# Chrixtar/latentsplat

Hardware: AMD Instinct MI355X
Metric: rendered target views/sec at 256x256, ~300k Gaussians (forward); fwd+bwd ms/view in `fwdbwd` (higher is better)
Workload: dtype f32; 1 GPU; BASELINE configs[1]: 300000 latent Gaussians (4-ch features + opacity), 256x256, forward render; 16 views of one scene per step per GPU; gaussians=300000, parallelism=replicas x1 (one scene per rank, no data-path collective)

## Files before the change

### latentsplat_amd/csrc/binning.hip

```cpp
#include "lsr_blend.h"
#include "lsr_tile_scan.h"
#include <algorithm>
#include <mutex>
#ifdef LSR_ENABLE_TRACE
#include <cstdio>
#include <cstdlib>
#include <vector>
#endif

namespace lsr {

constexpr int kScanThreads = 1024;

constexpr int kScanRegs = 8;

__global__ void __launch_bounds__(kScanThreads)
k_tile_scan(const uint32_t *__restrict__ count, uint32_t *__restrict__ start, uint32_t *header,
            uint32_t *host_words, uint32_t host_seq, uint32_t *__restrict__ order, int N, uint32_t capacity) {
    __shared__ TileScanShared<kScanThreads> s_scan;
    tile_scan_block<kScanThreads, kScanRegs, false>(count, start, header, HostMirror{host_words, host_seq}, order, N, capacity, s_scan);
}

hipError_t launch_tile_scan(const lsr_dims &d, char *geom, uint32_t *host_words, uint32_t host_seq, uint32_t pair_capacity, hipStream_t s) {
    const GeomLayout L = geom_layout(d);
// ... 107 lines not shown
    if (trace && threadIdx.x == 0) {
        unsigned hwid, xcc;
        asm volatile("s_getreg_b32 %0, hwreg(HW_REG_HW_ID)" : "=s"(hwid));
        asm volatile("s_getreg_b32 %0, hwreg(HW_REG_XCC_ID)" : "=s"(xcc));
        trace[8 * (size_t)blockIdx.x + 7] = ((unsigned long long)(xcc & 0xff) << 32) | hwid;
    }
#endif
#undef LSR_STAMP
}

constexpr int kSortThreads = 512;

struct HalfOut {
    uint32_t *half_list, *half_count;
    uint32_t *header;
    uint32_t capacity;
    uint32_t *long_list;
    uint32_t long_cap;
    uint32_t *long_count[2];
    IndexPacking ip;
    uint32_t seg_cap;
    const uint64_t *seg_keys;
    uint32_t n_limit;
};
constexpr int kSortTier2 = 8192;
__device__ __forceinline__ uint32_t long_tile(const HalfOut &ho, int cls, uint32_t i) {
    return ho.long_list[cls ? ho.long_cap - 1u - i : i];
}
__device__ __forceinline__ uint32_t key_index(const HalfOut &ho, uint32_t low_word) { return low_word >> ho.ip.key_shift; }
__device__ __forceinline__ uint32_t key_mask(const HalfOut &ho, uint32_t low_word) { return ho.ip.key_shift ? code_mask(low_word & 0xFFu) : 0xFFFFu; }
__device__ __forceinline__ uint32_t list_entry(const HalfOut &ho, uint32_t idx, uint32_t bits) { return idx | ((bits << kListBitsShift) & ~ho.ip.index_mask); }
constexpr int kEmitTab = 130;

template <int THREADS, class LowWord>
__device__ __forceinline__ void emit_half_lists(const HalfOut &ho, uint32_t n, uint32_t *hdst, uint32_t *hcnt, uint64_t *s_tab, LowWord low_word) {
    const int tid = threadIdx.x, lane = tid & (LSR_WAVE - 1), wid = tid / LSR_WAVE;
    constexpr int kWaves = THREADS / LSR_WAVE;
    uint32_t run0 = 0u, run1 = 0u;
    for (uint32_t base = 0; base < n; base += LSR_WAVE * LSR_WAVE) {
        for (int c = wid; c < LSR_WAVE; c += kWaves) {
            const uint32_t p = base + (uint32_t)(c * LSR_WAVE + lane);
            uint64_t packed = 0;
            if (p - lane < n) {
                const uint32_t w = low_word(min(p, n - 1));
                const uint32_t m16 = p < n ? key_mask(ho, w) : 0u;
                packed = (uint64_t)__builtin_popcountll(__ballot((m16 & 0x00FFu) != 0u)) |
                         ((uint64_t)__builtin_popcountll(__ballot((m16 & 0xFF00u) != 0u)) << 32);
            }
            if (lane == 0) s_tab[c] = packed;
        }
        __syncthreads();
        if (wid == 0) {
            const uint64_t v = s_tab[lane];
            uint64_t incl = v;
#pragma unroll
            for (int off = 1; off < LSR_WAVE; off <<= 1) { const uint64_t t = __shfl_up(incl, off); if (lane >= off) incl += t; }
            s_tab[LSR_WAVE + lane] = incl - v;
            if (lane == LSR_WAVE - 1) s_tab[2 * LSR_WAVE] = incl;
        }
        __syncthreads();
        const uint64_t tot = s_tab[2 * LSR_WAVE];
        for (int c = wid; c < LSR_WAVE; c += kWaves) {
            const uint32_t p = base + (uint32_t)(c * LSR_WAVE + lane);
            if (p - lane >= n) break;
            const uint32_t w = low_word(min(p, n - 1));
            const uint32_t idx = key_index(ho, w), m16 = p < n ? key_mask(ho, w) : 0u;
            const uint64_t off = s_tab[LSR_WAVE + c];
#pragma unroll
            for (int h = 0; h < 2; ++h) {
                const uint32_t bits = half_bits(m16, h);
                const uint64_t bal = __ballot(bits != 0u);
                if (bits) {
                    const uint32_t below = __builtin_amdgcn_mbcnt_hi((uint32_t)(bal >> 32), __builtin_amdgcn_mbcnt_lo((uint32_t)bal, 0u));
                    hdst[(size_t)h * n + (h ? run1 : run0) + (uint32_t)(off >> (32 * h)) + below] = list_entry(ho, idx, bits);
                }
            }
        }
        run0 += (uint32_t)tot; run1 += (uint32_t)(tot >> 32);
        __syncthreads();
    }
    if (tid < 2) hcnt[tid] = tid == 0 ? run0 : run1;
}

constexpr uint32_t kBucketOverflow = 48;

template <int CAP, int THREADS>
__device__ __forceinline__ void sort_tile(uint64_t *s_keys, size_t vt, int tier, const uint32_t *__restrict__ tile_start,
                                          const uint64_t *__restrict__ keys, uint32_t *__restrict__ point_list,
                                          const HalfOut &ho, unsigned long long *trace) {
#ifdef LSR_ENABLE_TRACE
#define LSR_STAMP(k) do { if (trace && threadIdx.x == 0) trace[8 * (size_t)blockIdx.x + (k)] = wall_clock64(); } while (0)
#else
#define LSR_STAMP(k) do { } while (0)
#endif
    LSR_STAMP(0);
    static_assert(CAP % THREADS == 0, "whole keys per thread");
    constexpr int NB = CAP < 2048 ? CAP : 2048;
    constexpr int kWaves = THREADS / LSR_WAVE;
    uint32_t *s_cnt = (uint32_t *)(s_keys + CAP);
    uint64_t *s_red = s_keys;
    uint32_t *s_wsum = (uint32_t *)(s_keys + 2 * kWaves);
    uint32_t *s_flag = s_wsum + kWaves;
    const int tid = threadIdx.x, lane = tid & (LSR_WAVE - 1), wid = tid / LSR_WAVE;
    const uint32_t start = tile_start[vt], n = tile_start[vt + 1] - start;
    uint32_t *hcnt = ho.half_count + 2 * vt, *hdst = ho.half_list + 2 * (size_t)start;
    if (n == 0) { if (tid < 2) hcnt[tid] = 0; return; }
    if ((uint64_t)start + n > ho.capacity) {
        if (tid < 2) hcnt[tid] = 0;
        if (tid == 0) ho.header[kHdrOverflow] = 1u;
        return;
    }
    if (n > ho.n_limit) {
        if (tid < 2) hcnt[tid] = 0;
        return;
    }
    if (n > (uint32_t)CAP) {
        if (tid == 0 && tier == 0) {
            const int cls = n > (uint32_t)kSortTier2 ? 1 : 0;
            const uint32_t i = atomicAdd(ho.long_count[cls], 1u);
            ho.long_list[cls ? ho.long_cap - 1u - i : i] = (uint32_t)vt;
        }
        return;
    }
    const uint64_t *src = (ho.seg_cap && n <= ho.seg_cap) ? ho.seg_keys + vt * (size_t)ho.seg_cap : keys + start;
    if (n == 1) {
        if (tid == 0) {
            const uint32_t w = (uint32_t)src[0], idx = key_index(ho, w);
            point_list[start] = idx;
            const uint32_t m = key_mask(ho, w);
            for (int h = 0; h < 2; ++h) {
                const uint32_t bits = half_bits(m, h);
                if (bits) hdst[h] = list_entry(ho, idx, bits);
                hcnt[h] = bits ? 1u : 0u;
            }
        }
        return;
    }

    constexpr int PERK = CAP / THREADS;
    uint64_t kreg[PERK];
#pragma unroll
    for (int q = 0; q < PERK; ++q) {
        const uint32_t i = tid + q * THREADS;
        const uint64_t k = src[min(i, n - 1)];
        kreg[q] = i < n ? k : ~0ull;
    }
    uint64_t kmin = ~0ull, kmax = 0ull;
#pragma unroll
    for (int q = 0; q < PERK; ++q) {
        const uint64_t k = kreg[q];
        kmin = k < kmin ? k : kmin;
        if (tid + q * THREADS < n) kmax = k > kmax ? k : kmax;
    }
#pragma unroll
    for (int off = 32; off > 0; off >>= 1) {
        const uint64_t a = __shfl_xor(kmin, off), b = __shfl_xor(kmax, off);
        kmin = a < kmin ? a : kmin; kmax = b > kmax ? b : kmax;
    }
    if (lane == 0) { s_red[2 * wid] = kmin; s_red[2 * wid + 1] = kmax; }
// ... 49 lines not shown
        for (int q = 0; q < PERK; ++q) {
            dst[q] = 0;
            if (tid + q * THREADS < n) {
                const uint64_t key = kreg[q];
                const uint32_t b = (uint32_t)((key - kmin) >> shift);
                const uint32_t lo = s_cnt[b], hi = b + 1 < (uint32_t)NB ? s_cnt[b + 1] : n;
                uint32_t below = 0;
                for (uint32_t j = lo; j < hi; j += 4) {
                    const uint32_t last = hi - 1;
                    const uint64_t m0 = s_keys[j], m1 = s_keys[min(j + 1, last)], m2 = s_keys[min(j + 2, last)], m3 = s_keys[min(j + 3, last)];
                    below += (m0 < key) + (j + 1 < hi && m1 < key) + (j + 2 < hi && m2 < key) + (j + 3 < hi && m3 < key);
                }
                dst[q] = lo + below;
            }
        }
        __syncthreads();
        uint32_t *s_out = (uint32_t *)s_keys;
#pragma unroll
        for (int q = 0; q < PERK; ++q)
            if (tid + q * THREADS < n) s_out[dst[q]] = (uint32_t)kreg[q];
        __syncthreads();
        LSR_STAMP(5);
        for (uint32_t i = tid; i < n; i += THREADS) point_list[start + i] = key_index(ho, s_out[i]);
        emit_half_lists<THREADS>(ho, n, hdst, hcnt, (uint64_t *)s_cnt, [&](uint32_t p) { return s_out[p]; });
        LSR_STAMP(6);
    } else {
        uint32_t npad = 2;
        while (npad < n) npad <<= 1;
        __syncthreads();
        if (npad <= (uint32_t)CAP) {
#pragma unroll
            for (int q = 0; q < PERK; ++q)
                if (tid + q * THREADS < npad) s_keys[tid + q * THREADS] = kreg[q];
        } else {
            static_assert(CAP * 8 + NB * 4 >= (CAP <= 2048 ? CAP : (CAP <= 4096 ? 4096 : CAP)) * 8, "bitonic padding fits the allocation");
#pragma unroll
            for (int q = 0; q < PERK; ++q) s_keys[tid + q * THREADS] = kreg[q];
            for (uint32_t i = CAP + tid; i < npad; i += THREADS) s_keys[i] = ~0ull;
        }
        __syncthreads();
        for (uint32_t k = 2; k <= npad; k <<= 1) {
            for (uint32_t j = k >> 1; j > 0; j >>= 1) {
                for (uint32_t t = tid; t < (npad >> 1); t += THREADS) {
                    const uint32_t lo = ((t & ~(j - 1)) << 1) | (t & (j - 1));
                    const uint32_t hi = lo | j;
                    const bool up = (lo & k) == 0;
                    const uint64_t a = s_keys[lo], b = s_keys[hi];
                    if ((a > b) == up) { s_keys[lo] = b; s_keys[hi] = a; }
                }
                __syncthreads();
            }
        }
        for (uint32_t i = tid; i < n; i += THREADS) point_list[start + i] = key_index(ho, (uint32_t)s_keys[i]);
        emit_half_lists<THREADS>(ho, n, hdst, hcnt, (uint64_t *)s_cnt, [&](uint32_t p) { return (uint32_t)s_keys[p]; });
    }
#ifdef LSR_ENABLE_TRACE
    if (trace && tid == 0) {
        unsigned hwid, xcc;
        asm volatile("s_getreg_b32 %0, hwreg(HW_REG_HW_ID)" : "=s"(hwid));
        asm volatile("s_getreg_b32 %0, hwreg(HW_REG_XCC_ID)" : "=s"(xcc));
        trace[8 * (size_t)blockIdx.x + 7] = ((unsigned long long)n << 40) | ((unsigned long long)(xcc & 0xff) << 32) | hwid;
    }
#endif
#undef LSR_STAMP
}

template <int CAP, int THREADS, bool PERSISTENT>
__global__ void __launch_bounds__(THREADS, CAP <= 4096 ? 6 : (CAP <= 8192 ? 4 : 2))
k_sort_tiles(int cls, const uint32_t *__restrict__ order, const uint32_t *__restrict__ tile_start, const uint64_t *__restrict__ keys,
             uint32_t *__restrict__ point_list, HalfOut ho, unsigned long long *trace) {
    extern __shared__ uint64_t s_keys[];
    if (!PERSISTENT) {
        const size_t vt = order ? (size_t)(order[2 * (size_t)blockIdx.x] & kItemTileMask) : (size_t)blockIdx.x;
        sort_tile<CAP, THREADS>(s_keys, vt, 0, tile_start, keys, point_list, ho, trace);
    } else {
        const uint32_t count = *ho.long_count[cls];
        for (uint32_t i = blockIdx.x; i < count; i += gridDim.x) {
            sort_tile<CAP, THREADS>(s_keys, long_tile(ho, cls, i), 1, tile_start, keys, point_list, ho, trace);
            __syncthreads();
        }
    }
}

__device__ __forceinline__ uint32_t lower_bound_u64(const uint64_t *a, uint32_t n, uint64_t x) {
    uint32_t lo = 0, hi = n;
    while (lo < hi) { const uint32_t mid = (lo + hi) >> 1; if (a[mid] < x) lo = mid + 1; else hi = mid; }
    return lo;
}
__device__ __forceinline__ void sort_tile_global(size_t vt, const uint32_t *__restrict__ tile_start, uint64_t *keys, uint64_t *tmp,
                                                 uint32_t *point_list, const HalfOut &ho, uint64_t *s_tab) {
    const uint32_t start = tile_start[vt], n = tile_start[vt + 1] - start;
    uint64_t *src = keys + start, *dst = tmp + start;
    for (uint32_t w = 1; w < n; w <<= 1) {
        for (uint32_t i = threadIdx.x; i < n; i += kSortThreads) {
            const uint32_t pair = i / (2 * w), a0 = pair * 2 * w;
            const uint32_t a1 = min(a0 + w, n), b1 = min(a0 + 2 * w, n);
            const uint64_t x = src[i];
            uint32_t pos;
            if (i < a1) pos = a0 + (i - a0) + lower_bound_u64(src + a1, b1 - a1, x);
            else pos = a0 + (i - a1) + lower_bound_u64(src + a0, a1 - a0, x);
            dst[pos] = x;
        }
        __threadfence_block();
        __syncthreads();
        uint64_t *t = src; src = dst; dst = t;
    }
    for (uint32_t i = threadIdx.x; i < n; i += kSortThreads)
        point_list[start + i] = key_index(ho, (uint32_t)src[i]);
    const uint64_t *sorted = src;
    emit_half_lists<kSortThreads>(ho, n, ho.half_list + 2 * (size_t)start, ho.half_count + 2 * vt, s_tab, [&](uint32_t p) { return (uint32_t)sorted[p]; });
}
__global__ void __launch_bounds__(kSortThreads)
k_sort_tiles_global(const uint32_t *__restrict__ tile_start, uint64_t *keys, uint64_t *tmp, uint32_t *point_list, HalfOut ho) {
    __shared__ uint64_t s_tab[kEmitTab];
    const uint32_t count = *ho.long_count[1];
    for (uint32_t it = blockIdx.x; it < count; it += gridDim.x) {
        const size_t vt = long_tile(ho, 1, it);
        if (tile_start[vt + 1] - tile_start[vt] <= (uint32_t)kSortLdsMax) continue;
        sort_tile_global(vt, tile_start, keys, tmp, point_list, ho, s_tab);
        __syncthreads();
    }
}
__global__ void __launch_bounds__(kSortThreads, 2)
k_sort_tiles_long(const uint32_t *__restrict__ tile_start, uint64_t *keys, uint64_t *tmp, uint32_t *point_list, HalfOut ho) {
    extern __shared__ uint64_t s_keys[];
    const uint32_t c0 = *ho.long_count[0], c1 = *ho.long_count[1];
    for (uint32_t it = blockIdx.x; it < c0 + c1; it += gridDim.x) {
        const size_t vt = it < c0 ? long_tile(ho, 0, it) : long_tile(ho, 1, it - c0);
        if (tile_start[vt + 1] - tile_start[vt] <= (uint32_t)kSortLdsMax) sort_tile<kSortLdsMax, kSortThreads>(s_keys, vt, 1, tile_start, keys, point_list, ho, nullptr);
        else sort_tile_global(vt, tile_start, keys, tmp, point_list, ho, s_keys);
        __syncthreads();
    }
}

template <int CAP>
constexpr size_t sort_lds_bytes() { return (size_t)CAP * 8 + (size_t)(CAP < 2048 ? CAP : 2048) * 4; }
template <int CAP, int THREADS, bool PERS>
static void sort_launch(dim3 grid, hipStream_t s, int cls, const uint32_t *order, const uint32_t *ts, const uint64_t *keys,
                        uint32_t *plist, const HalfOut &ho, unsigned long long *trace) {
    constexpr size_t lds = sort_lds_bytes<CAP>();
    if (lds > 48 * 1024) {
        static uint64_t done = 0;
        static std::mutex mu;
        int dev = 0;
        (void)hipGetDevice(&dev);
        std::lock_guard<std::mutex> lock(mu);
        if (dev < 0 || dev >= 64 || !((done >> dev) & 1ull)) {
            (void)hipFuncSetAttribute((const void *)k_sort_tiles<CAP, THREADS, PERS>, hipFuncAttributeMaxDynamicSharedMemorySize, (int)lds);
            if (dev >= 0 && dev < 64) done |= 1ull << dev;
        }
    }
    hipLaunchKernelGGL((k_sort_tiles<CAP, THREADS, PERS>), grid, dim3(THREADS), lds, s, cls, order, ts, keys, plist, ho, trace);
}

hipError_t launch_binning(const lsr_dims &d, char *geom, char *bin, int64_t num_pairs,
                          int32_t max_tile_pairs, const int32_t *radii, hipStream_t s, bool device_counts, bool seg, bool speculative) {
    (void)radii;
    const GeomLayout L = geom_layout(d);
    if (num_pairs <= 0 || d.num_gaussians == 0)
        return launch_clear(geom + L.half_count, align_up((size_t)d.num_views * (size_t)num_tiles(d) * 8, 16), s);
    const BinLayout B = bin_layout(d, num_pairs, device_counts ? kSortLdsMax + 1 : max_tile_pairs);
    const int T = (int)num_tiles(d), gx = tiles_x(d);
    if (seg && L.seg_cap == 0) return hipErrorInvalidValue;
    uint64_t *keys = (uint64_t *)(bin + B.keys);
    uint32_t *plist = (uint32_t *)(bin + B.point_list);
    const uint32_t *ts = (const uint32_t *)(geom + L.tile_start);
    HalfOut ho;
    ho.half_list = (uint32_t *)(bin + B.half_list); ho.half_count = (uint32_t *)(geom + L.half_count);
    ho.header = (uint32_t *)(geom + L.header);
    ho.capacity = (uint32_t)(num_pairs < 0xFFFFFFFFll ? num_pairs : 0xFFFFFFFFll);
    ho.long_list = (uint32_t *)(geom + L.tile_cursor);
    ho.long_cap = (uint32_t)d.num_views * (uint32_t)T;
    ho.long_count[0] = ho.header + kHdrLongTiles; ho.long_count[1] = ho.long_count[0] + 1;
    ho.ip = index_packing(d);
    ho.seg_cap = seg ? L.seg_cap : 0u;
    ho.seg_keys = (const uint64_t *)(geom + L.seg_keys);
    ho.n_limit = speculative ? (uint32_t)max_tile_pairs : 0xFFFFFFFFu;
    const uint32_t over_cap = seg ? L.seg_cap : 0u;
    if (!seg || device_counts || (uint32_t)max_tile_pairs > L.seg_cap) {
        const bool lds = T <= 8192;
        const int64_t resident = (int64_t)device_cus() * (lds ? std::max<int64_t>(1, std::min<int64_t>(8, (160 * 1024) / ((int64_t)T * 8 + 64))) : 8);
        const int64_t work = (int64_t)d.num_views * d.num_gaussians;
        const int64_t rounds = (work + resident * kScatThreads * kScatItems - 1) / (resident * kScatThreads * kScatItems);
        int items = (int)((work + resident * kScatThreads * rounds - 1) / (resident * kScatThreads * rounds));
        const int min_items = (int)((d.num_gaussians + (int64_t)kScatThreads * 160 - 1) / ((int64_t)kScatThreads * 160));
        items = std::max(1, std::min(kScatItems, std::max(items, min_items)));
        const uint32_t chunks = (uint32_t)((d.num_gaussians + kScatThreads * items - 1) / (kScatThreads * items));
        dim3 grid(chunks * (uint32_t)d.num_views);
        unsigned long long *strace = nullptr;
#ifdef LSR_ENABLE_TRACE
        const char *strace_path = getenv("LSR_TRACE_SCATTER");
        if (strace_path) {
            (void)hipMalloc((void **)&strace, (size_t)grid.x * 64);
            (void)hipMemsetAsync(strace, 0, (size_t)grid.x * 64, s);
        }
#endif
        prof_begin(kStScatter, s);
        const uint32_t capacity = (uint32_t)(num_pairs < 0xFFFFFFFFll ? num_pairs : 0xFFFFFFFFll);
#define LSR_SCAT2(LDSR, NRW, SHM)                                                                         \
    hipLaunchKernelGGL((k_scatter<LDSR, NRW>), grid, dim3(kScatThreads), SHM, s, d.num_gaussians, gx, T, \
// ... 90 lines not shown
```

### latentsplat_amd/csrc/lsr_internal.h

```cpp
#pragma once
#include <hip/hip_runtime.h>
#include <stdint.h>

#include "lsr_rasterizer.h"

#if defined(__HIP_DEVICE_COMPILE__) && !defined(__gfx950__)
#error "liblsr_hip is written for gfx950 (MI355X / CDNA4) only: build with --offload-arch=gfx950"
#endif
#define LSR_WAVE 64
#define LSR_NEAR_CULL 0.2f
#define LSR_LOWPASS 0.3f
#define LSR_ALPHA_MAX 0.99f
#define LSR_ALPHA_MIN (1.0f / 255.0f)
#define LSR_T_EPS 0.0001f

namespace lsr {

inline size_t align_up(size_t x, size_t a = 256) { return (x + a - 1) / a * a; }

struct GeomLayout {
    size_t header, rec, bin, tile_count, tile_start, tile_cursor, item_flags, bin_queue, item_cost, tile_order2, tile_order, half_count, sh_clamp, seg_keys, total;
    int rec_floats;
    uint32_t seg_cap;
};
struct ImgLayout {
    size_t final_T, n_contrib, total;
};
struct BinLayout {
    size_t keys, point_list, half_list, tmp, total;
};
constexpr size_t kBinQueueBytes = 4096 * 4;
constexpr int kCostClasses = 1024;
constexpr uint32_t kMaxReorderItems = 16384;
struct GradLayout {
    size_t rec, fixed, total;
    int rec_floats;
};
inline int grad_rec_floats(const lsr_dims &d);

inline int tiles_x(const lsr_dims &d) { return (d.width + LSR_TILE - 1) / LSR_TILE; }
inline int tiles_y(const lsr_dims &d) { return (d.height + LSR_TILE - 1) / LSR_TILE; }
inline int64_t num_tiles(const lsr_dims &d) { return (int64_t)tiles_x(d) * tiles_y(d); }

inline int rec_floats(const lsr_dims &d) {
// ... 24 lines not shown
    uint32_t cap;
    uint32_t key_shift;
    uint32_t ablate;
};

inline GeomLayout geom_layout(const lsr_dims &d) {
    GeomLayout L;
    const size_t VG = (size_t)d.num_views * (size_t)d.num_gaussians;
    const size_t VT = (size_t)d.num_views * (size_t)num_tiles(d);
    size_t o = 0;
    L.rec_floats = rec_floats(d);
    L.rec = o; o = align_up(o + VG * (size_t)L.rec_floats * 4);
    L.bin = o; o = align_up(o + VG * bin_stride(d));
    L.header = o; o += 256;
    L.tile_count = o; o = align_up(o + VT * 4);
    L.tile_cursor = o; o = align_up(o + VT * 4);
    L.item_flags = o; o = align_up(o + 2 * VT * 4);
    L.bin_queue = o; o += kBinQueueBytes;
    L.tile_start = o; o = align_up(o + (VT + 1) * 4);
    L.tile_order = o; o = align_up(o + 2 * VT * 4);
    L.item_cost = o; o = align_up(o + 2 * VT * 4);
    L.tile_order2 = o; o = align_up(o + 2 * VT * 4);
    L.half_count = o; o = align_up(o + 2 * VT * 4);
    L.sh_clamp = o; o = align_up(o + VG);
    L.seg_cap = segment_capacity(d);
    L.seg_keys = o; o = align_up(o + VT * (size_t)L.seg_cap * 8);
    L.total = o;
    return L;
}
inline ImgLayout img_layout(const lsr_dims &d) {
    ImgLayout L;
    const size_t n = (size_t)d.num_views * d.height * d.width;
    L.final_T = 0;
    L.n_contrib = align_up(n * 4);
    L.total = L.n_contrib + align_up(n * 4);
    return L;
}
constexpr int kSortLdsMax = 16384;
inline BinLayout bin_layout(const lsr_dims &d, int64_t num_pairs, int32_t max_tile_pairs) {
    BinLayout L;
    const size_t P = (size_t)(num_pairs > 0 ? num_pairs : 1);
    L.keys = 0;
    L.point_list = align_up(P * 8);
    L.half_list = L.point_list + align_up(P * 4);
    L.tmp = L.half_list + align_up(P * 8);
    L.total = L.tmp + (max_tile_pairs > kSortLdsMax ? align_up(P * 8) : 0);
// ... 18 lines not shown

constexpr uint32_t kItemFlagSteep = 1u;
constexpr float kSteepOpacity = 0.75f;
constexpr uint32_t kItemTileMask = 0x0FFFFFFFu;
constexpr int kItemHalfShift = 28;
constexpr uint32_t kListIndexMask = 0x00FFFFFFu;
constexpr int kListBitsShift = 24;
constexpr int kMaxGaussians = 1 << 24;
struct IndexPacking {
    uint32_t key_shift;
    uint32_t index_mask;
    uint32_t all_bits;
};
__host__ __device__ inline bool reached_only(const lsr_dims &d) { return (d.forward_flags & LSR_FWD_REACHED_ONLY) != 0 && d.num_gaussians <= (1 << 24); }
inline IndexPacking index_packing(const lsr_dims &d) {
    return d.num_gaussians > kMaxGaussians ? IndexPacking{0u, 0xFFFFFFFFu, 0xFFu} : IndexPacking{(uint32_t)kKeyIndexShift, kListIndexMask, 0u};
}
int device_cus();
inline int wave_slots(int cus) { return cus * 4 * 4; }
int env_int(const char *name, int fallback);
enum { kHdrPairs = 0, kHdrMaxTile = 1, kHdrNumItems = 3, kHdrOverflow = 4, kHdrPreDone = 5,
       kHdrFlagsValid = 6 ,
       kHdrQueueFwd = 8, kHdrOrder2Valid = 9 ,
       kHdrLongTiles = 16  };

enum Stage { kStPreprocess = 0, kStTileScan, kStScatter, kStSort, kStRenderFwd, kStRenderBwd, kStPreprocessBwd, kStShFwd, kStShBwd, kStAdapterFwd, kStAdapterBwd, kStLatentFwd, kStLatentBwd, kStViewGrad, kNumStages };
void prof_begin(int stage, hipStream_t s);
void prof_end(int stage, hipStream_t s);
void note_hip_error(int hip_error);

hipError_t launch_clear(void *ptr, size_t bytes, hipStream_t s);

constexpr int kPreThreadsScan = 256, kFoldTiles = 4096;
struct FoldedScan {
    int enabled;
    uint32_t *host_words; uint32_t host_seq;
    uint32_t capacity;
    uint32_t *tile_start, *tile_order;
};
inline bool fold_tile_scan(const lsr_dims &d) {
    return d.num_gaussians > 0 && (int64_t)d.num_views * num_tiles(d) <= kFoldTiles && env_int("LSR_FOLD_SCAN", 1) != 0;
}
hipError_t launch_preprocess(const lsr_dims &d, const lsr_inputs &in, char *geom, int32_t *radii, const FoldedScan &fs,
                             bool seg, hipStream_t s);
hipError_t launch_tile_scan(const lsr_dims &d, char *geom, uint32_t *host_words, uint32_t host_seq, uint32_t pair_capacity, hipStream_t s);
hipError_t launch_pack_view(const float *viewmatrix, const float *projmatrix, const float *campos, const float *bg,
// ... 88 lines not shown
```

### latentsplat_amd/csrc/render_forward.hip

```cpp
#include <stdio.h>

#include <vector>

#include "lsr_blend.h"

namespace lsr {

__device__ __forceinline__ void wave_lds_fence() {
    asm volatile("" ::: "memory");
    __builtin_amdgcn_wave_barrier();
}

typedef float float2_t __attribute__((ext_vector_type(2)));


__device__ __forceinline__ float2_t pk_mul_nw(float2_t a, float2_t b) {
    float2_t d;
    asm("v_pk_mul_f32 %0, %1, %2" : "=v"(d) : "v"(a), "v"(b));
    return d;
}
__device__ __forceinline__ float2_t pk_fma_bhi_nw(float2_t a, float2_t b, float2_t c) {
    float2_t d;
    asm("v_pk_fma_f32 %0, %1, %2, %3 op_sel:[0,1,0]" : "=v"(d) : "v"(a), "v"(b), "v"(c));
    return d;
}
template <bool HI>
__device__ __forceinline__ void pk_fma_splat(float2_t &acc, float2_t src, float2_t ww) {
    if (HI) asm("v_pk_fma_f32 %0, %1, %2, %0 op_sel:[1,0,0]" : "+v"(acc) : "v"(src), "v"(ww));
    else asm("v_pk_fma_f32 %0, %1, %2, %0 op_sel_hi:[0,1,1]" : "+v"(acc) : "v"(src), "v"(ww));
}

struct RenderFwdParams {
    int H, W, gx, T, G, C, has_color;
    int num_cus;
    int waves_per_cu;
    const uint32_t *items;
    uint32_t num_items;
    uint32_t quad_items;
    uint32_t all_live;
    uint32_t *queue;
    uint32_t *bin_queue;
    const uint32_t *header;
    int prio_pct;
    unsigned long long *trace;
    const float *views;
    const float4 *rec;
    int rec_f4;
    const uint32_t *tile_start, *half_count, *half_list;
    uint32_t *half_list_rw;
    uint32_t *item_cost;
    uint32_t *item_flags;
    uint32_t *header_rw;
    IndexPacking ip;
    float *out_color, *out_feat, *out_mask, *out_depth;
    float *final_T;
    uint32_t *n_contrib;
};

template <int NCHP, int WPB, bool RECORD = false, int EMU = 0>
// ... 2 lines not shown
    constexpr int kEnt = (2 + NCHP / 4) | 1;
    struct Lds {
        float4 ent[WPB][LSR_WAVE + 1][kEnt];
        uint32_t list[WPB][8][LSR_WAVE + 1];
    };
    __shared__ Lds s_lds;

    const int lane = threadIdx.x & (LSR_WAVE - 1);
    const int wid = __builtin_amdgcn_readfirstlane(threadIdx.x / LSR_WAVE);
    float4 (*s_ent)[kEnt] = s_lds.ent[wid];
    uint32_t (*s_list)[LSR_WAVE + 1] = s_lds.list[wid];
    const char *ent_base = (const char *)&s_lds.ent[0][0][0];
    const uint32_t wave_off = (uint32_t)(wid * (LSR_WAVE + 1) * kEnt * 16);
    const uint32_t my_off = wave_off + (uint32_t)(lane * kEnt * 16);
    const uint32_t null_off = wave_off + (uint32_t)(LSR_WAVE * kEnt * 16);
    if (lane < 8) s_list[lane][LSR_WAVE] = null_off;
    if (lane == 0) {
        s_ent[LSR_WAVE][0] = make_float4(__builtin_nanf(""), 0.0f, 0.0f, 0.0f);
        s_ent[LSR_WAVE][1] = make_float4(0.0f, 0.0f, 0.0f, RECORD ? 0.0f : -kInv255);
#pragma unroll
        for (int c4 = 0; c4 < NCHP / 4; ++c4) s_ent[LSR_WAVE][2 + c4] = make_float4(0.0f, 0.0f, 0.0f, 0.0f);
    }
    constexpr uint32_t kEmu = EMU ? (uint32_t)EMU : 1u;
    const uint32_t num_items = p.num_items * kEmu;
    const int coff = p.has_color ? 3 : 0;
    float2_t kz2 = float2_t{-kInv255, -kInv255};
    asm volatile("" : "+s"(kz2));
    const uint32_t gbit = 1u << (lane >> 3);
    const size_t HW = (size_t)p.H * p.W;
    const int grp = lane >> 3, gcol = grp & 3, grow = grp >> 2;
    const int lx = 2 * (lane & 1), ly = (lane >> 1) & 3;

    const uint32_t simd_bins = (uint32_t)p.num_cus * 4u, slots = (uint32_t)p.num_cus * (uint32_t)p.waves_per_cu;
    const uint32_t vwave = (uint32_t)wid + (uint32_t)WPB * (blockIdx.x / (uint32_t)p.num_cus);
    uint32_t prio_target = p.prio_pct ? (uint32_t)(((uint64_t)p.header[kHdrPairs] * (uint32_t)p.prio_pct) / (50ull * (uint64_t)max(num_items, 1u))) : 0u;
    if (prio_target < 3u * LSR_WAVE) prio_target = 0u;
    const uint32_t bin = (blockIdx.x % (uint32_t)p.num_cus) * 4u + (vwave & 3u);
    const uint32_t j0 = vwave >> 2;
    bool first = true;
    for (;;) {
        uint32_t qi;
        if (first) {
            qi = (j0 & 1u) ? (j0 + 1u) * simd_bins - 1u - bin : j0 * simd_bins + bin;
            first = false;
            if (qi >= num_items) continue;
        } else {
            if (num_items <= slots) break;
            uint32_t t = 0;
            if (p.bin_queue) {
                if (lane == 0) t = atomicAdd(p.bin_queue + bin, 1u);
                const uint32_t k = (uint32_t)p.waves_per_cu / 4u + __builtin_amdgcn_readfirstlane(t);
                qi = (k & 1u) ? (k + 1u) * simd_bins - 1u - bin : k * simd_bins + bin;
            } else {
                if (lane == 0) t = atomicAdd(p.queue, 1u);
                qi = slots + __builtin_amdgcn_readfirstlane(t);
            }
            if (qi >= num_items) break;
        }
#ifdef LSR_ENABLE_TRACE
        const unsigned long long t_begin = p.trace ? __builtin_readcyclecounter() : 0ull;
        unsigned long long t_first = 0ull, t_loop = 0ull;
        uint32_t trace_iters = 0;
#endif
        qi = __builtin_amdgcn_readfirstlane(qi);
        const uint32_t item = p.items[qi / kEmu];
        const uint32_t vt = item & kItemTileMask, half = item >> kItemHalfShift;
        const int tile = (int)(vt % (uint32_t)p.T), v = (int)(vt / (uint32_t)p.T);
        const int tx0 = (tile % p.gx) * LSR_TILE, ty0 = (tile / p.gx) * LSR_TILE + 8 * (int)half;
        const size_t vG = (size_t)v * p.G;
        const uint32_t tstart = p.tile_start[vt], tn = p.tile_start[vt + 1] - tstart;
        uint32_t hn = p.half_count[2 * (size_t)vt + half];
        const uint32_t *hlist = p.half_list + 2 * (size_t)tstart + (size_t)half * tn;
        if (EMU) {
            const uint32_t nbat = (hn + LSR_WAVE - 1) / LSR_WAVE, part = qi % kEmu;
            const uint32_t b0 = part * nbat / kEmu, b1 = (part + 1u) * nbat / kEmu;
            hlist += b0 * LSR_WAVE;
            hn = min(hn, b1 * LSR_WAVE) - min(hn, b0 * LSR_WAVE);
        }

        const int px = tx0 + 4 * gcol + lx, py = ty0 + 4 * grow + ly;
        const bool inside0 = px < p.W && py < p.H, inside1 = px + 1 < p.W && py < p.H;
        float2_t pxx = float2_t{inside0 ? (float)px : __builtin_nanf(""), inside1 ? (float)(px + 1) : __builtin_nanf("")};
        const float pyf = (float)py;
        float2_t T2 = float2_t{1.0f, 1.0f};
        float2_t D2 = float2_t{0.0f, 0.0f};
        float2_t acc[NCHP];
#pragma unroll
        for (int c = 0; c < NCHP; ++c) acc[c] = float2_t{0.0f, 0.0f};
// ... 662 lines not shown
        uint32_t list[WPB][4 * (LSR_WAVE + 1)];
    };
    __shared__ Lds s_lds;
    SmallWave<NCHP> w;
    w.lane = threadIdx.x & (LSR_WAVE - 1);
    const int lane = w.lane;
    const int wid = __builtin_amdgcn_readfirstlane(threadIdx.x / LSR_WAVE);
    w.s_ent = s_lds.ent[wid];
    w.s_flat = s_lds.list[wid];
    w.ent_base = (const char *)&s_lds.ent[0][0][0];
    w.wave_off = (uint32_t)(wid * (LSR_WAVE + 1) * kEnt * 16);
    w.my_off = w.wave_off + (uint32_t)(lane * kEnt * 16);
    w.null_off = w.wave_off + (uint32_t)(LSR_WAVE * kEnt * 16);
    w.coff = p.has_color ? 3 : 0;
    w.HW = (size_t)p.H * p.W;
    if (lane < 4) w.s_flat[lane * (LSR_WAVE + 1) + LSR_WAVE] = w.null_off;
    if (lane == 0) {
        w.s_ent[LSR_WAVE][0] = make_float4(__builtin_nanf(""), 0.0f, 0.0f, 0.0f);
        w.s_ent[LSR_WAVE][1] = make_float4(0.0f, 0.0f, 0.0f, -kInv255);
#pragma unroll
        for (int c4 = 0; c4 < NCHP / 4; ++c4) w.s_ent[LSR_WAVE][2 + c4] = make_float4(0.0f, 0.0f, 0.0f, 0.0f);
    }
    const uint32_t quad_end = 8u * p.quad_items;
    const uint32_t num_items = quad_end + 2u * (p.num_items - p.quad_items);

    const uint32_t simd_bins = (uint32_t)p.num_cus * 4u, slots = (uint32_t)p.num_cus * (uint32_t)p.waves_per_cu;
    const uint32_t vwave = (uint32_t)wid + (uint32_t)WPB * (blockIdx.x / (uint32_t)p.num_cus);
    const uint32_t bin = (blockIdx.x % (uint32_t)p.num_cus) * 4u + (vwave & 3u);
    const uint32_t j0 = vwave >> 2;
    bool first = true;
    for (;;) {
        uint32_t qi;
        if (first) {
            qi = (j0 & 1u) ? (j0 + 1u) * simd_bins - 1u - bin : j0 * simd_bins + bin;
            first = false;
            if (qi >= num_items) continue;
        } else {
            if (num_items <= slots) break;
            uint32_t t = 0;
            if (lane == 0) t = atomicAdd(p.queue, 1u);
            qi = slots + __builtin_amdgcn_readfirstlane(t);
            if (qi >= num_items) break;
        }
        qi = __builtin_amdgcn_readfirstlane(qi);
        if (qi == 0u && lane == 0) p.header_rw[kHdrFlagsValid] = 1u;
        if (qi < quad_end) {
            render_subblock_item<NCHP>(p, w, p.items[qi >> 3], (int)(qi & 7u));
        } else {
            const uint32_t r = qi - quad_end;
            render_row_item<NCHP, REC>(p, w, p.items[p.quad_items + (r >> 1)], (int)(r & 1u));
        }
    }
}

hipError_t launch_render_forward(const lsr_dims &d, const lsr_inputs &in, const char *geom,
                                 const char *bin, int64_t num_pairs, char *img, const lsr_outputs &out,
                                 hipStream_t s) {
    const GeomLayout L = geom_layout(d);
    const ImgLayout I = img_layout(d);
    const BinLayout B = bin_layout(d, num_pairs, 0);
    RenderFwdParams p;
    p.H = d.height; p.W = d.width; p.gx = tiles_x(d); p.T = (int)num_tiles(d); p.G = d.num_gaussians;
    p.C = d.feat_channels; p.has_color = d.color_mode != LSR_COLOR_NONE;
    p.num_cus = device_cus();
    p.items = (const uint32_t *)(geom + L.tile_order);
    p.num_items = 2u * (uint32_t)d.num_views * (uint32_t)p.T;
    p.queue = (uint32_t *)(geom + L.header) + kHdrQueueFwd;
    p.bin_queue = nullptr;
    p.header = (const uint32_t *)(geom + L.header); p.prio_pct = 0;
    p.views = in.views;
    p.rec = (const float4 *)(geom + L.rec); p.rec_f4 = L.rec_floats / 4;
    p.tile_start = (const uint32_t *)(geom + L.tile_start);
    p.half_count = (const uint32_t *)(geom + L.half_count);
    p.half_list = (const uint32_t *)(bin + B.half_list);
    p.half_list_rw = (uint32_t *)(const_cast<char *>(bin) + B.half_list);
    p.item_cost = nullptr;
    p.item_flags = (uint32_t *)(const_cast<char *>(geom) + L.item_flags);
    p.header_rw = (uint32_t *)(const_cast<char *>(geom) + L.header);
    p.ip = index_packing(d);
    p.out_color = out.color; p.out_feat = out.feature; p.out_mask = out.mask; p.out_depth = out.depth;
    p.final_T = (float *)(img + I.final_T); p.n_contrib = (uint32_t *)(img + I.n_contrib);
    const int nch = (p.has_color ? 3 : 0) + d.feat_channels;
    const int nchp = nch <= 4 ? 4 : (nch <= 8 ? 8 : (nch <= 12 ? 12 : 36));

    p.trace = nullptr;
    p.quad_items = 0;
    p.all_live = env_int("LSR_FWD_LIVE", 1) == 0 ? 1u : 0u;
#ifdef LSR_ENABLE_TRACE
// ... 85 lines not shown
```

Before: 40720 views/s.

## Order forward render items by exact per-half-tile cost computed during sort

During tile sorting, each half-tile's render cost is computed from the emitted per-entry bit masks (wave-level max popcount per 8 sub-blocks). The last sorting block to finish, detected via an atomic counter, counting-sorts all items by descending cost and writes an exact forward work order. The forward renderer uses that order when a header flag is set. The aim is better load balance in the persistent render queue, at the cost of extra work in the sort kernels and a serial ordering tail in one block. The tail also relies on relaxed cross-block atomics for correctness.

```diff
diff --git a/latentsplat_amd/csrc/binning.hip b/latentsplat_amd/csrc/binning.hip
--- a/latentsplat_amd/csrc/binning.hip
+++ b/latentsplat_amd/csrc/binning.hip
@@ -153,6 +153,9 @@
     uint32_t seg_cap;
     const uint64_t *seg_keys;
     uint32_t n_limit;
+    uint32_t *fwd_cost;
+    uint32_t *order_fwd;
+    uint32_t num_tiles;
 };
 constexpr int kSortTier2 = 8192;
 __device__ __forceinline__ uint32_t long_tile(const HalfOut &ho, int cls, uint32_t i) {
@@ -164,9 +167,13 @@
 constexpr int kEmitTab = 130;
 
 template <int THREADS, class LowWord>
-__device__ __forceinline__ void emit_half_lists(const HalfOut &ho, uint32_t n, uint32_t *hdst, uint32_t *hcnt, uint64_t *s_tab, LowWord low_word) {
+__device__ __forceinline__ void emit_half_lists(const HalfOut &ho, uint32_t n, uint32_t *hdst, uint32_t *hcnt, uint64_t *s_tab, LowWord low_word,
+                                                uint8_t *s_bits, uint32_t &cost0, uint32_t &cost1) {
     const int tid = threadIdx.x, lane = tid & (LSR_WAVE - 1), wid = tid / LSR_WAVE;
     constexpr int kWaves = THREADS / LSR_WAVE;
+    const bool costs = ho.fwd_cost != nullptr;
+    uint32_t *s_cost = (uint32_t *)(s_tab + kEmitTab - 1);
+    if (tid < 2) s_cost[tid] = 0u;
     uint32_t run0 = 0u, run1 = 0u;
     for (uint32_t base = 0; base < n; base += LSR_WAVE * LSR_WAVE) {
         for (int c = wid; c < LSR_WAVE; c += kWaves) {
@@ -203,7 +210,9 @@
                 const uint64_t bal = __ballot(bits != 0u);
                 if (bits) {
                     const uint32_t below = __builtin_amdgcn_mbcnt_hi((uint32_t)(bal >> 32), __builtin_amdgcn_mbcnt_lo((uint32_t)bal, 0u));
-                    hdst[(size_t)h * n + (h ? run1 : run0) + (uint32_t)(off >> (32 * h)) + below] = list_entry(ho, idx, bits);
+                    const uint32_t at = (h ? run1 : run0) + (uint32_t)(off >> (32 * h)) + below;
+                    hdst[(size_t)h * n + at] = list_entry(ho, idx, bits);
+                    if (costs && s_bits) s_bits[h * n + at] = (uint8_t)bits;
                 }
             }
         }
@@ -211,14 +220,121 @@
         __syncthreads();
     }
     if (tid < 2) hcnt[tid] = tid == 0 ? run0 : run1;
+    cost0 = cost1 = 0u;
+    if (!costs) return;
+    if (!s_bits) { __threadfence_block(); __syncthreads(); }
+    const uint32_t nb0 = (run0 + LSR_WAVE - 1) / LSR_WAVE, nb1 = (run1 + LSR_WAVE - 1) / LSR_WAVE;
+    uint32_t sum0 = 0u, sum1 = 0u;
+    for (uint32_t b = wid; b < nb0 + nb1; b += kWaves) {
+        const uint32_t h = b >= nb0 ? 1u : 0u, e = (h ? b - nb0 : b) * LSR_WAVE + lane, hn = h ? run1 : run0;
+        uint32_t m = 0u;
+        if (e < hn) m = s_bits ? (uint32_t)s_bits[h * n + e] : (((hdst[(size_t)h * n + e] >> kListBitsShift) | ho.ip.all_bits) & 0xFFu);
+        uint32_t nk = 0u;
+#pragma unroll
+        for (int g = 0; g < 8; ++g) nk = max(nk, (uint32_t)__builtin_popcountll(__ballot((m >> g) & 1u)));
+        if (h) sum1 += nk; else sum0 += nk;
+    }
+    if (lane == 0) {
+        if (sum0) atomicAdd(&s_cost[0], sum0);
+        if (sum1) atomicAdd(&s_cost[1], sum1);
+    }
+    __syncthreads();
+    cost0 = s_cost[0]; cost1 = s_cost[1];
+}
+
+constexpr int kOrderScratch = 32 + kCostClasses;
+template <int THREADS>
+__device__ __forceinline__ void order_items(const HalfOut &ho, uint32_t *s_ord) {
+    const int tid = threadIdx.x, lane = tid & (LSR_WAVE - 1), wid = tid / LSR_WAVE;
+    constexpr int kWaves = THREADS / LSR_WAVE, kPer = kMaxReorderItems / THREADS, kCls = kCostClasses / THREADS;
+    static_assert(kCostClasses % THREADS == 0 && kMaxReorderItems % (4 * THREADS) == 0 && kWaves <= 16, "whole classes / items per thread");
+    const uint32_t num_items = 2u * ho.num_tiles;
+    uint32_t *s_wsum = s_ord + 8, *s_cnt = s_ord + 32;
+    for (int b = tid; b < kCostClasses; b += THREADS) s_cnt[b] = 0u;
+    if (tid == 0) s_ord[1] = 0u;
+    constexpr int kRound = kPer / 4;
+    uint32_t c2[kPer / 2], mx = 0u;
+#pragma unroll
+    for (int q = 0; q < kPer / 2; ++q) c2[q] = 0u;
+#pragma unroll
+    for (int r = 0; r < 4; ++r) {
+        if (num_items > (uint32_t)(r * kRound * THREADS)) {
+            uint32_t c[kRound];
+#pragma unroll
+            for (int q = 0; q < kRound; ++q)
+                c[q] = __hip_atomic_load(&ho.fwd_cost[(uint32_t)tid + (uint32_t)(r * kRound + q) * THREADS], __ATOMIC_RELAXED, __HIP_MEMORY_SCOPE_AGENT);
+#pragma unroll
+            for (int q = 0; q < kRound; ++q) {
+                const uint32_t i = (uint32_t)tid + (uint32_t)(r * kRound + q) * THREADS;
+                const uint32_t v = i < num_items ? min(c[q], 0xFFFFu) : 0u;
+                mx = max(mx, v);
+                c2[(r * kRound + q) / 2] |= v << (16 * (q & 1));
+            }
+            __builtin_amdgcn_sched_barrier(0);
+        }
+    }
+#pragma unroll
+    for (int off = 32; off > 0; off >>= 1) mx = max(mx, (uint32_t)__shfl_xor(mx, off));
+    __syncthreads();
+    if (lane == 0) atomicMax(&s_ord[1], mx);
+    __syncthreads();
+    mx = s_ord[1];
+    const uint32_t shift = mx >= (uint32_t)kCostClasses ? (uint32_t)(32 - __builtin_clz(mx)) - 10u : 0u;
+    const uint32_t top = ((uint32_t)kCostClasses - 1u) * 0x00010001u, keep = (0xFFFFu >> shift) * 0x00010001u;
+#pragma unroll
+    for (int q = 0; q < kPer / 2; ++q) c2[q] = top - ((c2[q] >> shift) & keep);
+    auto class_of = [&](int q) -> uint32_t {
+        uint32_t w = c2[q / 2];
+        asm volatile("" : "+v"(w));
+        return (w >> (16 * (q & 1))) & 0xFFFFu;
+    };
+#pragma unroll
+    for (int q = 0; q < kPer; ++q) {
+        if ((uint32_t)tid + (uint32_t)q * THREADS < num_items) atomicAdd(&s_cnt[class_of(q)], 1u);
+        if ((q & 3) == 3) __builtin_amdgcn_sched_barrier(0);
+    }
+    __syncthreads();
+    uint32_t loc[kCls], sum = 0u;
+#pragma unroll
+    for (int k = 0; k < kCls; ++k) { loc[k] = s_cnt[tid * kCls + k]; sum += loc[k]; }
+    uint32_t incl = sum;
+#pragma unroll
+    for (int off = 1; off < LSR_WAVE; off <<= 1) { const uint32_t t = __shfl_up(incl, off); if (lane >= off) incl += t; }
+    if (lane == LSR_WAVE - 1) s_wsum[wid] = incl;
+    __syncthreads();
+    uint32_t run = incl - sum;
+#pragma unroll
+    for (int w = 0; w < kWaves; ++w) run += w < wid ? s_wsum[w] : 0u;
+#pragma unroll
+    for (int k = 0; k < kCls; ++k) { s_cnt[tid * kCls + k] = run; run += loc[k]; }
+    __syncthreads();
+#pragma unroll
+    for (int q = 0; q < kPer; ++q) {
+        const uint32_t i = (uint32_t)tid + (uint32_t)q * THREADS;
+        if (i < num_items) ho.order_fwd[atomicAdd(&s_cnt[class_of(q)], 1u)] = (i >> 1) | ((i & 1u) << kItemHalfShift);
+        if ((q & 3) == 3) __builtin_amdgcn_sched_barrier(0);
+    }
+    if (tid == 0) ho.header[kHdrOrderFwdValid] = 1u;
+}
+template <int THREADS>
+__device__ __forceinline__ bool tile_done(const HalfOut &ho, size_t vt, uint32_t cost0, uint32_t cost1, uint32_t *s_ord) {
+    if (!ho.fwd_cost) return false;
+    if (threadIdx.x == 0) {
+        __hip_atomic_store(&ho.fwd_cost[2 * vt], cost0, __ATOMIC_RELAXED, __HIP_MEMORY_SCOPE_AGENT);
+        __hip_atomic_store(&ho.fwd_cost[2 * vt + 1], cost1, __ATOMIC_RELAXED, __HIP_MEMORY_SCOPE_AGENT);
+        asm volatile("s_waitcnt vmcnt(0)" ::: "memory");
+        s_ord[0] = __hip_atomic_fetch_add(&ho.header[kHdrSortDone], 1u, __ATOMIC_RELAXED, __HIP_MEMORY_SCOPE_AGENT);
+    }
+    __syncthreads();
+    return s_ord[0] + 1u == ho.num_tiles;
 }
 
 constexpr uint32_t kBucketOverflow = 48;
 
 template <int CAP, int THREADS>
-__device__ __forceinline__ void sort_tile(uint64_t *s_keys, size_t vt, int tier, const uint32_t *__restrict__ tile_start,
+__device__ __forceinline__ bool sort_tile(uint64_t *s_keys, size_t vt, int tier, const uint32_t *__restrict__ tile_start,
                                           const uint64_t *__restrict__ keys, uint32_t *__restrict__ point_list,
-                                          const HalfOut &ho, unsigned long long *trace) {
+                                          const HalfOut &ho, unsigned long long *trace, uint32_t &cost0, uint32_t &cost1) {
 #ifdef LSR_ENABLE_TRACE
 #define LSR_STAMP(k) do { if (trace && threadIdx.x == 0) trace[8 * (size_t)blockIdx.x + (k)] = wall_clock64(); } while (0)
 #else
@@ -235,15 +351,16 @@
     const int tid = threadIdx.x, lane = tid & (LSR_WAVE - 1), wid = tid / LSR_WAVE;
     const uint32_t start = tile_start[vt], n = tile_start[vt + 1] - start;
     uint32_t *hcnt = ho.half_count + 2 * vt, *hdst = ho.half_list + 2 * (size_t)start;
-    if (n == 0) { if (tid < 2) hcnt[tid] = 0; return; }
+    cost0 = cost1 = 0u;
+    if (n == 0) { if (tid < 2) hcnt[tid] = 0; return true; }
     if ((uint64_t)start + n > ho.capacity) {
         if (tid < 2) hcnt[tid] = 0;
         if (tid == 0) ho.header[kHdrOverflow] = 1u;
-        return;
+        return true;
     }
     if (n > ho.n_limit) {
         if (tid < 2) hcnt[tid] = 0;
-        return;
+        return true;
     }
     if (n > (uint32_t)CAP) {
         if (tid == 0 && tier == 0) {
@@ -251,7 +368,7 @@
             const uint32_t i = atomicAdd(ho.long_count[cls], 1u);
             ho.long_list[cls ? ho.long_cap - 1u - i : i] = (uint32_t)vt;
         }
-        return;
+        return false;
     }
     const uint64_t *src = (ho.seg_cap && n <= ho.seg_cap) ? ho.seg_keys + vt * (size_t)ho.seg_cap : keys + start;
     if (n == 1) {
@@ -263,9 +380,10 @@
                 const uint32_t bits = half_bits(m, h);
                 if (bits) hdst[h] = list_entry(ho, idx, bits);
                 hcnt[h] = bits ? 1u : 0u;
+                (h ? cost1 : cost0) = bits ? 1u : 0u;
             }
         }
-        return;
+        return true;
     }
 
     constexpr int PERK = CAP / THREADS;
@@ -361,8 +479,7 @@
         __syncthreads();
         LSR_STAMP(5);
         for (uint32_t i = tid; i < n; i += THREADS) point_list[start + i] = key_index(ho, s_out[i]);
-        emit_half_lists<THREADS>(ho, n, hdst, hcnt, (uint64_t *)s_cnt, [&](uint32_t p) { return s_out[p]; });
-        LSR_STAMP(6);
+        emit_half_lists<THREADS>(ho, n, hdst, hcnt, (uint64_t *)s_cnt, [&](uint32_t p) { return s_out[p]; }, (uint8_t *)(s_out + n), cost0, cost1);
     } else {
         uint32_t npad = 2;
         while (npad < n) npad <<= 1;
@@ -391,8 +508,9 @@
             }
         }
         for (uint32_t i = tid; i < n; i += THREADS) point_list[start + i] = key_index(ho, (uint32_t)s_keys[i]);
-        emit_half_lists<THREADS>(ho, n, hdst, hcnt, (uint64_t *)s_cnt, [&](uint32_t p) { return (uint32_t)s_keys[p]; });
-    }
+        emit_half_lists<THREADS>(ho, n, hdst, hcnt, (uint64_t *)s_cnt, [&](uint32_t p) { return (uint32_t)s_keys[p]; }, nullptr, cost0, cost1);
+    }
+    LSR_STAMP(6);
 #ifdef LSR_ENABLE_TRACE
     if (trace && tid == 0) {
         unsigned hwid, xcc;
@@ -402,6 +520,7 @@
     }
 #endif
 #undef LSR_STAMP
+    return true;
 }
 
 template <int CAP, int THREADS, bool PERSISTENT>
@@ -411,13 +530,19 @@
     extern __shared__ uint64_t s_keys[];
     if (!PERSISTENT) {
         const size_t vt = order ? (size_t)(order[2 * (size_t)blockIdx.x] & kItemTileMask) : (size_t)blockIdx.x;
-        sort_tile<CAP, THREADS>(s_keys, vt, 0, tile_start, keys, point_list, ho, trace);
+        uint32_t c0, c1;
+        if (sort_tile<CAP, THREADS>(s_keys, vt, 0, tile_start, keys, point_list, ho, trace, c0, c1) && tile_done<THREADS>(ho, vt, c0, c1, (uint32_t *)s_keys))
+            order_items<THREADS>(ho, (uint32_t *)s_keys);
     } else {
         const uint32_t count = *ho.long_count[cls];
+        bool last = false;
         for (uint32_t i = blockIdx.x; i < count; i += gridDim.x) {
-            sort_tile<CAP, THREADS>(s_keys, long_tile(ho, cls, i), 1, tile_start, keys, point_list, ho, trace);
+            const size_t vt = long_tile(ho, cls, i);
+            uint32_t c0, c1;
+            if (sort_tile<CAP, THREADS>(s_keys, vt, 1, tile_start, keys, point_list, ho, trace, c0, c1)) last |= tile_done<THREADS>(ho, vt, c0, c1, (uint32_t *)s_keys);
             __syncthreads();
         }
+        if (last) order_items<THREADS>(ho, (uint32_t *)s_keys);
     }
 }
 
@@ -426,7 +551,8 @@
     while (lo < hi) { const uint32_t mid = (lo + hi) >> 1; if (a[mid] < x) lo = mid + 1; else hi = mid; }
     return lo;
 }
-__device__ __forceinline__ void sort_tile_global(size_t vt, const uint32_t *__restrict__ tile_start, uint64_t *keys, uint64_t *tmp,
+constexpr int kGlobalTab = kEmitTab > (kOrderScratch + 1) / 2 ? kEmitTab : (kOrderScratch + 1) / 2;
+__device__ __forceinline__ bool sort_tile_global(size_t vt, const uint32_t *__restrict__ tile_start, uint64_t *keys, uint64_t *tmp,
                                                  uint32_t *point_list, const HalfOut &ho, uint64_t *s_tab) {
     const uint32_t start = tile_start[vt], n = tile_start[vt + 1] - start;
     uint64_t *src = keys + start, *dst = tmp + start;
@@ -447,29 +573,38 @@
     for (uint32_t i = threadIdx.x; i < n; i += kSortThreads)
         point_list[start + i] = key_index(ho, (uint32_t)src[i]);
     const uint64_t *sorted = src;
-    emit_half_lists<kSortThreads>(ho, n, ho.half_list + 2 * (size_t)start, ho.half_count + 2 * vt, s_tab, [&](uint32_t p) { return (uint32_t)sorted[p]; });
+    uint32_t c0, c1;
+    emit_half_lists<kSortThreads>(ho, n, ho.half_list + 2 * (size_t)start, ho.half_count + 2 * vt, s_tab, [&](uint32_t p) { return (uint32_t)sorted[p]; },
+                                  nullptr, c0, c1);
+    return tile_done<kSortThreads>(ho, vt, c0, c1, (uint32_t *)s_tab);
 }
 __global__ void __launch_bounds__(kSortThreads)
 k_sort_tiles_global(const uint32_t *__restrict__ tile_start, uint64_t *keys, uint64_t *tmp, uint32_t *point_list, HalfOut ho) {
-    __shared__ uint64_t s_tab[kEmitTab];
+    __shared__ uint64_t s_tab[kGlobalTab];
     const uint32_t count = *ho.long_count[1];
+    bool last = false;
     for (uint32_t it = blockIdx.x; it < count; it += gridDim.x) {
         const size_t vt = long_tile(ho, 1, it);
         if (tile_start[vt + 1] - tile_start[vt] <= (uint32_t)kSortLdsMax) continue;
-        sort_tile_global(vt, tile_start, keys, tmp, point_list, ho, s_tab);
-        __syncthreads();
-    }
+        last |= sort_tile_global(vt, tile_start, keys, tmp, point_list, ho, s_tab);
+        __syncthreads();
+    }
+    if (last) order_items<kSortThreads>(ho, (uint32_t *)s_tab);
 }
 __global__ void __launch_bounds__(kSortThreads, 2)
 k_sort_tiles_long(const uint32_t *__restrict__ tile_start, uint64_t *keys, uint64_t *tmp, uint32_t *point_list, HalfOut ho) {
     extern __shared__ uint64_t s_keys[];
     const uint32_t c0 = *ho.long_count[0], c1 = *ho.long_count[1];
+    bool last = false;
     for (uint32_t it = blockIdx.x; it < c0 + c1; it += gridDim.x) {
         const size_t vt = it < c0 ? long_tile(ho, 0, it) : long_tile(ho, 1, it - c0);
-        if (tile_start[vt + 1] - tile_start[vt] <= (uint32_t)kSortLdsMax) sort_tile<kSortLdsMax, kSortThreads>(s_keys, vt, 1, tile_start, keys, point_list, ho, nullptr);
-        else sort_tile_global(vt, tile_start, keys, tmp, point_list, ho, s_keys);
-        __syncthreads();
-    }
+        uint32_t k0, k1;
+        if (tile_start[vt + 1] - tile_start[vt] <= (uint32_t)kSortLdsMax) {
+            if (sort_tile<kSortLdsMax, kSortThreads>(s_keys, vt, 1, tile_start, keys, point_list, ho, nullptr, k0, k1)) last |= tile_done<kSortThreads>(ho, vt, k0, k1, (uint32_t *)s_keys);
+        } else last |= sort_tile_global(vt, tile_start, keys, tmp, point_list, ho, s_keys);
+        __syncthreads();
+    }
+    if (last) order_items<kSortThreads>(ho, (uint32_t *)s_keys);
 }
 
 template <int CAP>
@@ -515,6 +650,10 @@
     ho.seg_cap = seg ? L.seg_cap : 0u;
     ho.seg_keys = (const uint64_t *)(geom + L.seg_keys);
     ho.n_limit = speculative ? (uint32_t)max_tile_pairs : 0xFFFFFFFFu;
+    ho.num_tiles = (uint32_t)d.num_views * (uint32_t)T;
+    const bool exact_order = 2u * ho.num_tiles <= kMaxReorderItems && env_int("LSR_FWD_EXACT_ORDER", 1) != 0;
+    ho.fwd_cost = exact_order ? (uint32_t *)(geom + L.fwd_cost) : nullptr;
+    ho.order_fwd = (uint32_t *)(geom + L.tile_order_fwd);
     const uint32_t over_cap = seg ? L.seg_cap : 0u;
     if (!seg || device_counts || (uint32_t)max_tile_pairs > L.seg_cap) {
         const bool lds = T <= 8192;
diff --git a/latentsplat_amd/csrc/lsr_internal.h b/latentsplat_amd/csrc/lsr_internal.h
--- a/latentsplat_amd/csrc/lsr_internal.h
+++ b/latentsplat_amd/csrc/lsr_internal.h
@@ -19,7 +19,7 @@
 inline size_t align_up(size_t x, size_t a = 256) { return (x + a - 1) / a * a; }
 
 struct GeomLayout {
-    size_t header, rec, bin, tile_count, tile_start, tile_cursor, item_flags, bin_queue, item_cost, tile_order2, tile_order, half_count, sh_clamp, seg_keys, total;
+    size_t header, rec, bin, tile_count, tile_start, tile_cursor, item_flags, bin_queue, item_cost, tile_order2, tile_order, half_count, fwd_cost, tile_order_fwd, sh_clamp, seg_keys, total;
     int rec_floats;
     uint32_t seg_cap;
 };
@@ -90,6 +90,8 @@
     L.item_cost = o; o = align_up(o + 2 * VT * 4);
     L.tile_order2 = o; o = align_up(o + 2 * VT * 4);
     L.half_count = o; o = align_up(o + 2 * VT * 4);
+    L.fwd_cost = o; o = align_up(o + (2 * VT > kMaxReorderItems ? 2 * VT : (size_t)kMaxReorderItems) * 4);
+    L.tile_order_fwd = o; o = align_up(o + 2 * VT * 4);
     L.sh_clamp = o; o = align_up(o + VG);
     L.seg_cap = segment_capacity(d);
     L.seg_keys = o; o = align_up(o + VT * (size_t)L.seg_cap * 8);
@@ -154,6 +156,8 @@
 enum { kHdrPairs = 0, kHdrMaxTile = 1, kHdrNumItems = 3, kHdrOverflow = 4, kHdrPreDone = 5,
        kHdrFlagsValid = 6 ,
        kHdrQueueFwd = 8, kHdrOrder2Valid = 9 ,
+       kHdrSortDone = 10 ,
+       kHdrOrderFwdValid = 11 ,
        kHdrLongTiles = 16  };
 
 enum Stage { kStPreprocess = 0, kStTileScan, kStScatter, kStSort, kStRenderFwd, kStRenderBwd, kStPreprocessBwd, kStShFwd, kStShBwd, kStAdapterFwd, kStAdapterBwd, kStLatentFwd, kStLatentBwd, kStViewGrad, kNumStages };
diff --git a/latentsplat_amd/csrc/render_forward.hip b/latentsplat_amd/csrc/render_forward.hip
--- a/latentsplat_amd/csrc/render_forward.hip
+++ b/latentsplat_amd/csrc/render_forward.hip
@@ -35,6 +35,7 @@
     int num_cus;
     int waves_per_cu;
     const uint32_t *items;
+    const uint32_t *items_exact;
     uint32_t num_items;
     uint32_t quad_items;
     uint32_t all_live;
@@ -83,6 +84,7 @@
         for (int c4 = 0; c4 < NCHP / 4; ++c4) s_ent[LSR_WAVE][2 + c4] = make_float4(0.0f, 0.0f, 0.0f, 0.0f);
     }
     constexpr uint32_t kEmu = EMU ? (uint32_t)EMU : 1u;
+    const uint32_t *items = p.header[kHdrOrderFwdValid] ? p.items_exact : p.items;
     const uint32_t num_items = p.num_items * kEmu;
     const int coff = p.has_color ? 3 : 0;
     float2_t kz2 = float2_t{-kInv255, -kInv255};
@@ -124,7 +126,7 @@
         uint32_t trace_iters = 0;
 #endif
         qi = __builtin_amdgcn_readfirstlane(qi);
-        const uint32_t item = p.items[qi / kEmu];
+        const uint32_t item = items[qi / kEmu];
         const uint32_t vt = item & kItemTileMask, half = item >> kItemHalfShift;
         const int tile = (int)(vt % (uint32_t)p.T), v = (int)(vt / (uint32_t)p.T);
         const int tx0 = (tile % p.gx) * LSR_TILE, ty0 = (tile / p.gx) * LSR_TILE + 8 * (int)half;
@@ -833,6 +835,7 @@
         for (int c4 = 0; c4 < NCHP / 4; ++c4) w.s_ent[LSR_WAVE][2 + c4] = make_float4(0.0f, 0.0f, 0.0f, 0.0f);
     }
     const uint32_t quad_end = 8u * p.quad_items;
+    const uint32_t *items = p.header[kHdrOrderFwdValid] ? p.items_exact : p.items;
     const uint32_t num_items = quad_end + 2u * (p.num_items - p.quad_items);
 
     const uint32_t simd_bins = (uint32_t)p.num_cus * 4u, slots = (uint32_t)p.num_cus * (uint32_t)p.waves_per_cu;
@@ -856,10 +859,10 @@
         qi = __builtin_amdgcn_readfirstlane(qi);
         if (qi == 0u && lane == 0) p.header_rw[kHdrFlagsValid] = 1u;
         if (qi < quad_end) {
-            render_subblock_item<NCHP>(p, w, p.items[qi >> 3], (int)(qi & 7u));
+            render_subblock_item<NCHP>(p, w, items[qi >> 3], (int)(qi & 7u));
         } else {
             const uint32_t r = qi - quad_end;
-            render_row_item<NCHP, REC>(p, w, p.items[p.quad_items + (r >> 1)], (int)(r & 1u));
+            render_row_item<NCHP, REC>(p, w, items[p.quad_items + (r >> 1)], (int)(r & 1u));
         }
     }
 }
@@ -875,6 +878,7 @@
     p.C = d.feat_channels; p.has_color = d.color_mode != LSR_COLOR_NONE;
     p.num_cus = device_cus();
     p.items = (const uint32_t *)(geom + L.tile_order);
+    p.items_exact = (const uint32_t *)(geom + L.tile_order_fwd);
     p.num_items = 2u * (uint32_t)d.num_views * (uint32_t)p.T;
     p.queue = (uint32_t *)(geom + L.header) + kHdrQueueFwd;
     p.bin_queue = nullptr;
```

Measured after the change: 39520 views/s. -3.0%, worse.
